# cambrian-mllm/cambrian

Measured on NVIDIA H100. Metric: train_samples_per_sec, higher is better.
Workload: dtype bf16

## Files before the change

cambrian_b200/autograd.py:

```python
from __future__ import annotations

import torch

from . import ops


def _ranged(tag):
    def deco(fn):
        def wrapped(*a, **k):
            with ops.nvtx(tag):
                return fn(*a, **k)
        wrapped.__name__ = fn.__name__
        wrapped.__doc__ = fn.__doc__
        return wrapped
    return deco


def _notify(param):
    n = getattr(param, "_cb_notify", None)
    if n is not None:
        n()


def _await(*params):
# ... 372 lines not shown
        ops.gemm(b, weight[:, D:], out=t32, accumulate=True)
        y = ops.f32_to_bf16(t32, torch.empty(t32.shape, dtype=torch.bfloat16, device=a.device))
        ctx.save_for_backward(a, b, weight)
        ctx.param = weight
        return y

    @staticmethod
    def backward(ctx, dy):
        a, b, weight = ctx.saved_tensors
        D = a.shape[1]
        dy = dy.contiguous()
        da = ops.gemm(dy, weight[:, :D], b_mn=True) if ctx.needs_input_grad[0] else None
        db = ops.gemm(dy, weight[:, D:], b_mn=True) if ctx.needs_input_grad[1] else None
        dw = None
        w_param = ctx.param
        if ctx.needs_input_grad[2] and not _frozen(w_param):
            if getattr(w_param, "main_grad", None) is not None:
                wgrad(w_param, dy, a, out_view=_slice_a(D), notify=False)
                wgrad(w_param, dy, b, out_view=_slice_b(D))
            else:
                dw = torch.cat([ops.gemm(dy, a, a_mn=True, b_mn=True), ops.gemm(dy, b, a_mn=True, b_mn=True)], 1)
        return da, db, dw


class LinearResidualFn(torch.autograd.Function):

    @staticmethod
    def forward(ctx, x, weight, residual):
        _await(weight)
        ctx.save_for_backward(x, weight)
        ctx.param = weight
        return ops.gemm(x, weight, residual=residual.contiguous())

    @staticmethod
    def backward(ctx, dy):
        x, weight = ctx.saved_tensors
        dy = dy.contiguous()
        dx = ops.gemm(dy, weight, b_mn=True) if ctx.needs_input_grad[0] else None
        dw = wgrad(ctx.param, dy, x) if ctx.needs_input_grad[1] else None
        return dx, dw, (dy if ctx.needs_input_grad[2] else None)


class NarrowLinearFn(torch.autograd.Function):

    PAD = 8

    @staticmethod
    def forward(ctx, x, weight):
        _await(weight)
        T, K = weight.shape
        if T > NarrowLinearFn.PAD:
            raise ValueError(f"NarrowLinearFn: {T} output rows > {NarrowLinearFn.PAD}")
        wpad = torch.zeros((NarrowLinearFn.PAD, K), dtype=weight.dtype, device=weight.device)
        wpad[:T].copy_(weight)
        ctx.save_for_backward(x, wpad)
        ctx.param, ctx.T = weight, T
        return ops.gemm(x, wpad)

    @staticmethod
    def backward(ctx, dy):
        x, wpad = ctx.saved_tensors
        dy = dy.contiguous()
        dx = ops.gemm(dy, wpad, b_mn=True) if ctx.needs_input_grad[0] else None
        dw = None
        if ctx.needs_input_grad[1] and not _frozen(ctx.param):
            dw = vgrad(ctx.param, ops.gemm(dy, x, a_mn=True, b_mn=True)[:ctx.T].contiguous())
        return dx, dw


class TowerCombineFn(torch.autograd.Function):

    @staticmethod
    def forward(ctx, logits, q_in, *aggs):
        aggs = [a.contiguous() for a in aggs]
        logits = logits.contiguous()
        ctx.save_for_backward(logits, *aggs)
        return ops.tower_combine_fwd(logits, aggs, q_in.contiguous())

    @staticmethod
    def backward(ctx, dout):
        logits, *aggs = ctx.saved_tensors
        dout = dout.contiguous()
        daggs, dlogits = ops.tower_combine_bwd(logits, aggs, dout)
        return (dlogits if ctx.needs_input_grad[0] else None, dout, *daggs)


class CrossAttnTowerFn(torch.autograd.Function):

    NAMES = ("q_ln_w", "q_ln_b", "q_w", "k_ln_w", "k_ln_b", "k_w", "v_ln_w", "v_ln_b", "v_w", "o_w", "pos")

    @staticmethod
    def forward(ctx, meta, q_in, feat, *tensors):
        _await(*meta["params"])
        P = dict(zip(CrossAttnTowerFn.NAMES, tensors))
        r = meta["r"]
        N = q_in.shape[0]
        nat = meta["natural"]
        windowed = nat is None
        B, q_side = (N, 1) if windowed else nat
        side = 0 if windowed else r * q_side
        masks = None if meta["mask"] is None else [meta["mask"]]
        f2 = feat.reshape(-1, feat.shape[-1])
        qn, mq, rq = ops.layernorm_fwd(q_in, P["q_ln_w"], P["q_ln_b"], 1e-5, save_stats=True)
        Q = ops.gemm(qn, P["q_w"])
        kin, mean, rstd = ops.layernorm_fwd(f2, P["k_ln_w"], P["k_ln_b"], 1e-5, pos=P["pos"], side=side, r=r, save_stats=True)
        vin = ops.layernorm_fwd(f2, P["v_ln_w"], P["v_ln_b"], 1e-5, pos=P["pos"], side=side, r=r)
        K = ops.gemm(kin, P["k_w"])
        V = ops.gemm(vin, P["v_w"])
        A, lse = ops.sva_window_attn_fwd(Q, [K], [V], masks, [r], B, q_side, need_lse=True, windowed=windowed)
        out = ops.gemm(A, P["o_w"])
        ctx.meta = meta
        ctx.dims = (N, B, q_side, windowed, side, feat.shape)
        ctx.save_for_backward(q_in, f2, qn, mq, rq, Q, kin, vin, mean, rstd, K, V, A, lse, *tensors)
        return out

    @staticmethod
    def backward(ctx, dout):
        meta = ctx.meta
        r = meta["r"]
        N, B, q_side, windowed, side, fshape = ctx.dims
        sv = ctx.saved_tensors
        q_in, f2, qn, mq, rq, Q, kin, vin, mean, rstd, K, V, A, lse = sv[:14]
        P = dict(zip(CrossAttnTowerFn.NAMES, sv[14:]))
        prm = dict(zip(CrossAttnTowerFn.NAMES, meta["params"]))
        masks = None if meta["mask"] is None else [meta["mask"]]
        g = {}
        dout = dout.contiguous()
        dA = ops.gemm(dout, P["o_w"], b_mn=True)
        g["o_w"] = wgrad(prm["o_w"], dout, A)
        dQ, (dK,), (dV,) = ops.sva_window_attn_bwd(Q, A, dA, lse, [K], [V], masks, [r], B, q_side, windowed=windowed)
        dqn = ops.gemm(dQ, P["q_w"], b_mn=True)
        g["q_w"] = wgrad(prm["q_w"], dQ, qn)
        dq_in, dgq, dbq = ops.layernorm_bwd(dqn, q_in, P["q_ln_w"], mq, rq)
        g["q_ln_w"], g["q_ln_b"] = vgrad(prm["q_ln_w"], dgq), vgrad(prm["q_ln_b"], dbq)
        dkin = ops.gemm(dK, P["k_w"], b_mn=True)
        g["k_w"] = wgrad(prm["k_w"], dK, kin)
        dvin = ops.gemm(dV, P["v_w"], b_mn=True)
        g["v_w"] = wgrad(prm["v_w"], dV, vin)
        dxk, dgk, dbk = ops.layernorm_bwd(dkin, f2, P["k_ln_w"], mean, rstd, pos=P["pos"], side=side, r=r)
        dxv, dgv, dbv = ops.layernorm_bwd(dvin, f2, P["v_ln_w"], mean, rstd, pos=P["pos"], side=side, r=r, dres=dxk)
        g["k_ln_w"], g["k_ln_b"] = vgrad(prm["k_ln_w"], dgk), vgrad(prm["k_ln_b"], dbk)
        g["v_ln_w"], g["v_ln_b"] = vgrad(prm["v_ln_w"], dgv), vgrad(prm["v_ln_b"], dbv)
        dp = ops.pos_grad(dxv, dxv.shape[0] // (r * r), r, r) if windowed else ops.pos_grad(dxv, B, r * q_side, r)
        g["pos"] = vgrad(prm["pos"], dp)
        return (None, dq_in, dxv.view(fshape), *[g[n] for n in CrossAttnTowerFn.NAMES])


class DecoderLayerFn(torch.autograd.Function):
    _nvtx = "DecoderLayer"

    """x [B,S,H] -> x'.  Parameters: input_ln, qkv_w (fused [ (nh+2nkv)*hd, H ]), o_w, post_ln, gu_w (fused [2I, H]), down_w.

    meta = dict(nh, nkv, hd, eps, hf_cast, cos, sin, pos (int64 [B*S]), kmask (bool [B,S] or None), params (6 Parameters),
                recompute (bool: keep only x and redo the forward in backward — per-layer activation checkpointing))
    """

    @staticmethod
    def _forward(meta, x, ln1, qkv_w, o_w, ln2, gu_w, down_w, keep, need_out=True):
        B, S, H = x.shape
        nh, nkv, hd = meta["nh"], meta["nkv"], meta["hd"]
        rows = B * S
        x2 = x.reshape(rows, H)
        h, rstd1 = ops.rmsnorm_fwd(x2, ln1, meta["eps"], meta["hf_cast"], save_stats=True)
        qkv = ops.gemm(h, qkv_w)
        ops.rope_(qkv, meta["pos"], meta["cos"], meta["sin"], nh + nkv, hd)
        q = qkv[:, : nh * hd].view(B, S, nh, hd)
        k = qkv[:, nh * hd:(nh + nkv) * hd].view(B, S, nkv, hd)
        v = qkv[:, (nh + nkv) * hd:].view(B, S, nkv, hd)
        attn, lse = ops.attn_fwd(q, k, v, causal=True, kmask=meta["kmask"], need_lse=True)
        attn2 = attn.view(rows, nh * hd)
        x1 = ops.gemm(attn2, o_w, residual=x2)
        h2, rstd2 = ops.rmsnorm_fwd(x1, ln2, meta["eps"], meta["hf_cast"], save_stats=True)
        gu, act = ops.mlp_gate_up(h2, gu_w)
        saved = (rstd1, qkv, attn, lse, x1, rstd2, gu, act) if keep else None
        if not need_out:
            return None, saved
        out = ops.gemm(act, down_w, residual=x1)
        return out.view(B, S, H), saved

    @staticmethod
    @_ranged("decoder_layer.fwd")
    def forward(ctx, meta, x, ln1, q_w, k_w, v_w, o_w, ln2, gate_w, up_w, down_w):
        keep = not meta["recompute"]
        _await(*meta["params"])
        qkv_w, gu_w = meta["qkv_w"], meta["gu_w"]
        out, saved = DecoderLayerFn._forward(meta, x, ln1, qkv_w, o_w, ln2, gu_w, down_w, keep)
        ctx.meta = meta
        if keep:
            ctx.save_for_backward(x, ln1, qkv_w, o_w, ln2, gu_w, down_w, *saved)
        else:
            ctx.save_for_backward(x, ln1, qkv_w, o_w, ln2, gu_w, down_w)
        return out

    @staticmethod
    @_ranged("decoder_layer.bwd")
    def backward(ctx, dout):
        meta = ctx.meta
        sv = ctx.saved_tensors
        x, ln1, qkv_w, o_w, ln2, gu_w, down_w = sv[:7]
        if meta["recompute"]:
            _, saved = DecoderLayerFn._forward(meta, x, ln1, qkv_w, o_w, ln2, gu_w, down_w, True, need_out=False)
        else:
            saved = sv[7:]
        rstd1, qkv, attn, lse, x1, rstd2, gu, act = saved
        p_ln1, p_qkv, p_o, p_ln2, p_gu, p_down = meta["params"]
        B, S, H = x.shape
        nh, nkv, hd = meta["nh"], meta["nkv"], meta["hd"]
        rows = B * S
        I = gu_w.shape[0] // 2
        x2 = x.reshape(rows, H)
        dx2 = dout.reshape(rows, H).contiguous()
        h2 = ops.rmsnorm_fwd(x1, ln2, meta["eps"], meta["hf_cast"])
        dact = ops.gemm(dx2, down_w, b_mn=True)
        g_down = wgrad(p_down, dx2, act)
        del act
        dgu = torch.empty_like(gu)
        ops.swiglu_bwd(dact, gu[:, :I], gu[:, I:], dgu[:, :I], dgu[:, I:])
        del dact
        dh2 = ops.gemm(dgu, gu_w, b_mn=True)
        g_gu = wgrad(p_gu, dgu, h2)
        del dgu, h2
        dx1, dg2 = ops.rmsnorm_bwd(dh2, x1, ln2, rstd2, dres=dx2)
        g_ln2 = vgrad(p_ln2, dg2)
        attn2 = attn.view(rows, nh * hd)
        dattn = ops.gemm(dx1, o_w, b_mn=True)
        g_o = wgrad(p_o, dx1, attn2)
        dqkv = torch.empty_like(qkv)
        q = qkv[:, : nh * hd].view(B, S, nh, hd)
        k = qkv[:, nh * hd:(nh + nkv) * hd].view(B, S, nkv, hd)
        v = qkv[:, (nh + nkv) * hd:].view(B, S, nkv, hd)
        ops.attn_bwd(q, k, v, attn, dattn.view(B, S, nh, hd), lse, causal=True, kmask=meta["kmask"],
                     dq=dqkv[:, : nh * hd].view(B, S, nh, hd), dk=dqkv[:, nh * hd:(nh + nkv) * hd].view(B, S, nkv, hd),
                     dv=dqkv[:, (nh + nkv) * hd:].view(B, S, nkv, hd))
        ops.rope_(dqkv, meta["pos"], meta["cos"], meta["sin"], nh + nkv, hd, inverse=True)
        h = ops.rmsnorm_fwd(x2, ln1, meta["eps"], meta["hf_cast"])
        dh = ops.gemm(dqkv, qkv_w, b_mn=True)
        g_qkv = wgrad(p_qkv, dqkv, h)
        del dqkv, h
        dx, dg1 = ops.rmsnorm_bwd(dh, x2, ln1, rstd1, dres=dx1)
        g_ln1 = vgrad(p_ln1, dg1)
        gq = gk = gv = gg = gup = None
        if g_qkv is not None:
            gq, gk, gv = g_qkv[: nh * hd], g_qkv[nh * hd:(nh + nkv) * hd], g_qkv[(nh + nkv) * hd:]
        if g_gu is not None:
            gg, gup = g_gu[:I], g_gu[I:]
        return None, dx.view(B, S, H), g_ln1, gq, gk, gv, g_o, g_ln2, gg, gup, g_down


class EmbedSpliceFn(torch.autograd.Function):

    @staticmethod
    def forward(ctx, meta, embed_w, img, newline):
        ids, img_start, q_side = meta["ids"], meta["img_start"], meta["q_side"]
        _await(*meta["params"])
        ctx.meta = meta
        ctx.has_img = img is not None
        ctx.vshape = embed_w.shape
        return ops.embed_splice(ids, img_start, embed_w, img, newline, q_side)

    @staticmethod
    def backward(ctx, dout):
        meta = ctx.meta
        p_embed, p_newline = meta["params"]
        dout = dout.contiguous()
        d_embed_ret = None
        tgt = None
        if ctx.needs_input_grad[1]:
            mg = getattr(p_embed, "main_grad", None)
            if mg is not None:
                fresh = getattr(p_embed, "_cb_fresh", None)
                if fresh is not None and "all" not in fresh:
                    mg.zero_()
                    fresh.add("all")
                tgt = mg
            else:
                tgt = torch.zeros(ctx.vshape, dtype=torch.bfloat16, device=dout.device)
                d_embed_ret = tgt
        d_img, d_nl_rows = ops.embed_splice_bwd(dout, meta["ids"], meta["img_start"], None, meta["q_side"], ctx.has_img)
        if tgt is not None:
            ops.embed_grad_sorted(dout, meta["ids"], meta["img_start"] if ctx.has_img else None, tgt, meta["q_side"])
        if tgt is not None and d_embed_ret is None:
            _notify(p_embed)
        d_nl = None
        if ctx.has_img and ctx.needs_input_grad[3]:
            d_nl = vgrad(p_newline, ops.group_colsum(d_nl_rows, 1).view(-1))
        return None, d_embed_ret, d_img, d_nl


class LMHeadLossFn(torch.autograd.Function):
    _nvtx = "LMHeadLoss"

    """cambrian_llama.py:402-422: lm_head -> logits.float() -> shift -> CrossEntropyLoss(mean over non-ignored), computed
    in row chunks so the [B*S, V] logits are never resident at once; the backward GEMMs run inside the forward (the
    per-chunk (softmax - onehot) overwrites the chunk's logits), so the only saved tensor is dhidden."""

    @staticmethod
    @_ranged("lm_head_loss.fwd")
    def forward(ctx, meta, hidden, weight):
        labels = meta["shift_labels"]
        rows, H = hidden.reshape(-1, hidden.shape[-1]).shape
        h2 = hidden.reshape(rows, H)
        V = weight.shape[0]
        dev = hidden.device
        chunk = meta.get("chunk", 4096)
        n_valid = meta["n_valid"]
        inv_dev = meta.get("inv_count_dev")
        train = meta["train"]
        p_w = meta["params"][0]
        _await(p_w)
        need_dw = train and not _frozen(p_w)
        ranges = meta.get("label_ranges")
        dh_full = None
        if ranges is not None:
            ranges = [(int(a), int(b)) for a, b in ranges if b > a]
            n_rows = sum(b - a for a, b in ranges)
            hc = torch.empty((max(n_rows, 1), H), dtype=h2.dtype, device=dev)
            lc = torch.full((max(n_rows, 1),), -100, dtype=labels.dtype, device=dev)
            o = 0
            for a, b in ranges:
                hc[o:o + b - a].copy_(h2[a:b])
                lc[o:o + b - a].copy_(labels[a:b])
                o += b - a
            if train:
                dh_full = torch.zeros_like(h2)
            h2, labels, rows = hc, lc, max(n_rows, 1)
        loss_rows = torch.empty(rows, dtype=torch.float32, device=dev)
        acc = torch.zeros(2, dtype=torch.float32, device=dev)
        dh = torch.empty_like(h2) if train else None
        gscale = float(meta.get("loss_scale", 1.0)) / (max(n_valid, 1) if n_valid is not None else 1)
        logits = torch.empty((min(chunk, rows), V), dtype=torch.bfloat16, device=dev)
        dw_local = None
        if need_dw and getattr(p_w, "main_grad", None) is None:
            dw_local = torch.empty_like(weight)
        for r0 in range(0, rows, chunk):
            r1 = min(rows, r0 + chunk)
            lg = logits[: r1 - r0]
            ops.gemm(h2[r0:r1], weight, out=lg)
            ops.cross_entropy(lg, labels[r0:r1], loss_rows[r0:r1], acc, gscale, train,
                              scale_dev=inv_dev if n_valid is None else None)
            if train:
                ops.gemm(lg, weight, b_mn=True, out=dh[r0:r1])
                if not need_dw:
                    pass
                elif dw_local is None:
                    wgrad(p_w, lg, h2[r0:r1], notify=False)
                else:
                    ops.gemm(lg, h2[r0:r1], a_mn=True, b_mn=True, out=dw_local, accumulate=r0 > 0)
        if need_dw and dw_local is None:
            _notify(p_w)
        if dh_full is not None:
            o = 0
            for a, b in ranges:
                dh_full[a:b].copy_(dh[o:o + b - a])
                o += b - a
            dh = dh_full
        ctx.train = train
        ctx.hshape = hidden.shape
# ... 69 lines not shown
```

cambrian_b200/csrc/attention.cu:

```cuda
#include "common.cuh"
#include <cudaTypedefs.h>
#include <type_traits>

namespace cb {

int make_tmap_bf16_4d(CUtensorMap* out, const void* base, uint64_t d0, uint64_t d1, uint64_t d2, uint64_t d3,
                      uint64_t s1, uint64_t s2, uint64_t s3, uint32_t box_rows);

constexpr float LOG2E = 1.4426950408889634f;

struct AttnParams {
  bf16* o;
  long long o_bs, o_ss;
  float* lse;
  const uint8_t* kmask;
  int B, nh, nkv, Sq, Skv, hd, causal;
  float scale_log2;
};

template <int N>
__device__ __forceinline__ bool keys_all_valid(const uint8_t* km, int k0) {
  constexpr int PER = N / 32;
  static_assert(PER == 2 || PER == 4, "64- or 128-key tiles");
  const uint8_t* kp = km + k0 + PER * (threadIdx.x & 31);
  uint32_t w = 0;
  if (!(reinterpret_cast<uintptr_t>(kp) & (PER - 1))) {
    w = PER == 4 ? *reinterpret_cast<const uint32_t*>(kp) : *reinterpret_cast<const uint16_t*>(kp);
  } else {
#pragma unroll
    for (int i = 0; i < PER; ++i) w |= (uint32_t)kp[i] << (8 * i);
  }
  bool ok = true;
#pragma unroll
  for (int i = 0; i < PER; ++i) ok = ok && ((w >> (8 * i)) & 0xffu);
  return __all_sync(0xffffffffu, ok);
}

struct TileIdx {
  int t, h, b;
};
__device__ __forceinline__ TileIdx tile_index(int heads, int B) {
  const int hb = heads * B;
  const int rem = (int)blockIdx.x % hb;
  return {(int)blockIdx.x / hb, rem % heads, rem / heads};
}

template <int HDP>
struct FwdCfg {
  static constexpr int ATOMS = (HDP + 63) / 64;
  static constexpr int TILE = ATOMS * 16384;
  static constexpr int STAGES = 3;
  static constexpr int SMEM = TILE * (1 + 2 * STAGES) + 1024 + 256;
};

template <int HDP>
__global__ void __launch_bounds__(288, 1)
attn_fwd_kernel(const __grid_constant__ CUtensorMap tmQ, const __grid_constant__ CUtensorMap tmK,
                const __grid_constant__ CUtensorMap tmV, AttnParams p) {
  using Cfg = FwdCfg<HDP>;
  constexpr int STAGES = Cfg::STAGES;
  extern __shared__ uint8_t smem_raw[];
  const uint32_t base = (smem_u32(smem_raw) + 1023u) & ~1023u;
  const uint32_t sQ = base;
  const uint32_t sK = sQ + Cfg::TILE;
  const uint32_t sV = sK + STAGES * Cfg::TILE;
  const uint32_t bars = sV + STAGES * Cfg::TILE;
  const uint32_t q_full = bars;
  auto k_full = [&](int s) { return bars + 8u * (1 + s); };
  auto v_full = [&](int s) { return bars + 8u * (1 + STAGES + s); };
  auto kv_empty = [&](int s) { return bars + 8u * (1 + 2 * STAGES + s); };

  const int warp = threadIdx.x >> 5, lane = threadIdx.x & 31;
  const int q_tiles = (p.Sq + 127) / 128;
  const TileIdx ti = tile_index(p.nh, p.B);
  const int qt = q_tiles - 1 - ti.t;
  const int h = ti.h, b = ti.b;
  const int hk = h / (p.nh / p.nkv);
  const int q0 = qt * 128;
  const int kv_tiles_all = (p.Skv + 127) / 128;
  const int coff = p.Skv - p.Sq;
  int n_tiles = kv_tiles_all;
  if (p.causal) {
    const int last_key = q0 + 127 + coff;
    n_tiles = min(kv_tiles_all, last_key / 128 + 1);
    if (n_tiles < 1) n_tiles = 1;
  }

  if (warp == 8 && lane == 0) {
    tma_prefetch_desc(&tmQ);
    tma_prefetch_desc(&tmK);
    tma_prefetch_desc(&tmV);
    mbar_init(q_full, 1);
    for (int s = 0; s < STAGES; ++s) {
      mbar_init(k_full(s), 1);
      mbar_init(v_full(s), 1);
      mbar_init(kv_empty(s), 2);
    }
    mbar_fence_init();
  }
  __syncthreads();

  if (warp == 8) {
    if (lane == 0) {
      mbar_arrive_expect_tx(q_full, Cfg::TILE);
#pragma unroll
      for (int a = 0; a < Cfg::ATOMS; ++a) tma_load_4d(sQ + a * 16384, &tmQ, q_full, a * 64, h, q0, b);
      int st = 0;
      uint32_t ph = 0;
      for (int j = 0; j < n_tiles; ++j) {
        mbar_wait(kv_empty(st), ph ^ 1u);
        mbar_arrive_expect_tx(k_full(st), Cfg::TILE);
#pragma unroll
        for (int a = 0; a < Cfg::ATOMS; ++a)
          tma_load_4d(sK + st * Cfg::TILE + a * 16384, &tmK, k_full(st), a * 64, hk, j * 128, b);
        mbar_arrive_expect_tx(v_full(st), Cfg::TILE);
#pragma unroll
        for (int a = 0; a < Cfg::ATOMS; ++a)
          tma_load_4d(sV + st * Cfg::TILE + a * 16384, &tmV, v_full(st), a * 64, hk, j * 128, b);
        if (++st == STAGES) { st = 0; ph ^= 1u; }
      }
    }
    return;
  }

  const int wg = warp >> 2;
  const bool wg_leader = (threadIdx.x & 127) == 0;
  const int rloc = wg * 64 + (warp & 3) * 16 + (lane >> 2);
  const int cq = 2 * (lane & 3);
  const uint8_t* km = p.kmask ? p.kmask + (size_t)b * p.Skv : nullptr;
  float o[HDP / 2];
#pragma unroll
  for (int i = 0; i < HDP / 2; ++i) o[i] = 0.f;
  float m_run[2] = {-INFINITY, -INFINITY}, l_run[2] = {0.f, 0.f};
  mbar_wait(q_full, 0);
  int st = 0;
  uint32_t ph = 0;
  for (int j = 0; j < n_tiles; ++j) {
    const int k0 = j * 128;
    float s[64];
    mbar_wait(k_full(st), ph);
    const uint32_t kb = sK + st * Cfg::TILE;
    wgmma_fence();
#pragma unroll
    for (int kk = 0; kk < HDP / 16; ++kk) {
      const uint32_t off = (kk >> 2) * 16384 + (kk & 3) * 32;
      WgmmaSS<128, 0, 0>::mma(s, make_smem_desc_sw128(sQ + wg * 8192 + off, 0, 1024),
                              make_smem_desc_sw128(kb + off, 0, 1024), kk ? 1u : 0u);
    }
    wgmma_commit();
    bool full_tile = k0 + 128 <= p.Skv && (!p.causal || k0 + 127 <= q0 + wg * 64 + coff);
    if (full_tile && km) full_tile = keys_all_valid<128>(km, k0);
    wgmma_wait<0>();
    reg_fence(s);
    float mx[2] = {-INFINITY, -INFINITY};
#pragma unroll
    for (int jj = 0; jj < 16; ++jj) {
#pragma unroll
      for (int e = 0; e < 4; ++e) {
        float v = s[4 * jj + e] * p.scale_log2;
        if (!full_tile) {
          const int key = k0 + 8 * jj + cq + (e & 1);
          const int qi = q0 + rloc + 8 * (e >> 1);
          const bool ok = key < p.Skv && (!p.causal || key <= qi + coff) && (!km || km[key]);
          v = ok ? v : -INFINITY;
        }
        s[4 * jj + e] = v;
        mx[e >> 1] = fmaxf(mx[e >> 1], v);
      }
    }
    float corr[2], mref[2];
#pragma unroll
    for (int r = 0; r < 2; ++r) {
      mx[r] = fmaxf(mx[r], __shfl_xor_sync(0xffffffffu, mx[r], 1));
      mx[r] = fmaxf(mx[r], __shfl_xor_sync(0xffffffffu, mx[r], 2));
      const float m_new = fmaxf(m_run[r], mx[r]);
      mref[r] = m_new == -INFINITY ? 0.f : m_new;
      corr[r] = fast_exp2(m_run[r] - mref[r]);
      m_run[r] = m_new;
      l_run[r] *= corr[r];
    }
#pragma unroll
    for (int jj = 0; jj < HDP / 8; ++jj) {
#pragma unroll
      for (int e = 0; e < 4; ++e) o[4 * jj + e] *= corr[e >> 1];
    }
    uint32_t pa[8][4];
#pragma unroll
    for (int jj = 0; jj < 16; ++jj) {
      float pv[4];
#pragma unroll
      for (int e = 0; e < 4; ++e) {
        pv[e] = fast_exp2(s[4 * jj + e] - mref[e >> 1]);
        l_run[e >> 1] += pv[e];
      }
      pa[jj >> 1][(jj & 1) * 2 + 0] = pack_bf16x2(pv[0], pv[1]);
      pa[jj >> 1][(jj & 1) * 2 + 1] = pack_bf16x2(pv[2], pv[3]);
    }
    mbar_wait(v_full(st), ph);
    const uint32_t vb = sV + st * Cfg::TILE;
    reg_fence(o);
    wgmma_fence();
#pragma unroll
    for (int kk = 0; kk < 8; ++kk)
      WgmmaRS<HDP, 1>::mma(o, pa[kk], make_smem_desc_sw128(vb + kk * 2048, 16384, 1024), 1u);
    wgmma_commit();
    wgmma_wait<0>();
    reg_fence(o);
    if (wg_leader) mbar_arrive(kv_empty(st));
    if (++st == STAGES) { st = 0; ph ^= 1u; }
  }
#pragma unroll
  for (int r = 0; r < 2; ++r) {
    float l = l_run[r];
    l += __shfl_xor_sync(0xffffffffu, l, 1);
    l += __shfl_xor_sync(0xffffffffu, l, 2);
    const int qi = q0 + rloc + 8 * r;
    if (qi >= p.Sq) continue;
    const float inv = l > 0.f ? 1.f / l : 0.f;
    bf16* op = p.o + (long long)b * p.o_bs + (long long)qi * p.o_ss + (long long)h * p.hd;
#pragma unroll
    for (int jj = 0; jj < HDP / 8; ++jj) {
      const int d = 8 * jj + cq;
      if (d < p.hd)
        *reinterpret_cast<__nv_bfloat162*>(op + d) = __floats2bfloat162_rn(o[4 * jj + 2 * r] * inv, o[4 * jj + 2 * r + 1] * inv);
    }
    if (p.lse && (lane & 3) == 0)
      p.lse[((long long)b * p.nh + h) * p.Sq + qi] = l > 0.f ? m_run[r] + log2f(l) : INFINITY;
  }
}

__global__ void attn_delta_kernel(const bf16* __restrict__ o, const bf16* __restrict__ d_o, float* __restrict__ delta,
                                  int B, int S, int nh, int hd, long long o_bs, long long o_ss, long long do_bs,
                                  long long do_ss) {
  const int lph = hd >> 3;
  const int hpw = 32 / lph;
  const long long w = (blockIdx.x * (long long)blockDim.x + threadIdx.x) >> 5;
  const int lane = threadIdx.x & 31;
  const long long total = (long long)B * S * nh;
  const long long idx = w * hpw + lane / lph;
  const int sub = lane % lph;
  float acc = 0.f;
  if (idx < total) {
    const int h = (int)(idx % nh);
    const long long t = idx / nh;
    const int s = (int)(t % S);
    const int b = (int)(t / S);
    const bf16* op = o + b * o_bs + s * o_ss + (long long)h * hd + sub * 8;
    const bf16* gp = d_o + b * do_bs + s * do_ss + (long long)h * hd + sub * 8;
    float a[8], g[8];
    unpack8(ldg_nc(op), a);
    unpack8(ldg_nc(gp), g);
#pragma unroll
    for (int e = 0; e < 8; ++e) acc += a[e] * g[e];
  }
  for (int off = lph >> 1; off > 0; off >>= 1) acc += __shfl_xor_sync(0xffffffffu, acc, off);
  if (idx < total && sub == 0) {
    const int h = (int)(idx % nh);
    const long long t = idx / nh;
    delta[((long long)(t / S) * nh + h) * S + (t % S)] = acc;
  }
}

struct AttnBwdParams {
  bf16* dq;
  bf16* dk;
  bf16* dv;
  long long dq_bs, dq_ss, dk_bs, dk_ss, dv_bs, dv_ss;
  const float* lse;
  const float* delta;
  const uint8_t* kmask;
  int B, nh, nkv, Sq, Skv, hd, causal;
  float scale_log2, scale;
};

template <int HDP>
struct BwdCfg {
  static constexpr int ATOMS = HDP / 64;
  static constexpr int KTILE = ATOMS * 16384;
  static constexpr int QTILE = ATOMS * 8192;
  static constexpr int STAGES = 4;
  static constexpr int SMEM = 2 * KTILE + 2 * STAGES * QTILE + STAGES * 512 + 1024 + 256;
};

template <int HDP>
__global__ void __launch_bounds__(384, 1)
attn_bwd_kernel(const __grid_constant__ CUtensorMap tmQ, const __grid_constant__ CUtensorMap tmK,
                const __grid_constant__ CUtensorMap tmV, const __grid_constant__ CUtensorMap tmdO, AttnBwdParams p) {
  using Cfg = BwdCfg<HDP>;
  constexpr int STAGES = Cfg::STAGES;
  extern __shared__ uint8_t smem_raw[];
  const uint32_t base = (smem_u32(smem_raw) + 1023u) & ~1023u;
  const uint32_t sK = base;
  const uint32_t sV = sK + Cfg::KTILE;
  const uint32_t sQ = sV + Cfg::KTILE;
  const uint32_t sdO = sQ + STAGES * Cfg::QTILE;
  const uint32_t sLD = sdO + STAGES * Cfg::QTILE;
  const uint32_t bars = sLD + STAGES * 512;
  const uint32_t kv_full = bars;
  auto qd_full = [&](int s) { return bars + 8u * (1 + s); };
  auto qd_empty = [&](int s) { return bars + 8u * (1 + STAGES + s); };
  float* ld_stage = reinterpret_cast<float*>(smem_raw + (sLD - smem_u32(smem_raw)));

  const int warp = threadIdx.x >> 5, lane = threadIdx.x & 31;
  const TileIdx ti = tile_index(p.nkv, p.B);
// ... 112 lines not shown
      for (int jj = 0; jj < 8; ++jj) {
        float pv[4], dsv[4];
#pragma unroll
        for (int c = 0; c < 2; ++c) {
          const int qc = 8 * jj + cq + c;
          const float L = ld[qc], D = ld[64 + qc];
#pragma unroll
          for (int r = 0; r < 2; ++r) {
            const int e = 2 * r + c;
            bool vis = true;
            if (!decltype(full_tile)::value)
              vis = qi0 + qc < p.Sq && key_ok[r] && (!p.causal || k0 + kr + 8 * r <= qi0 + qc + coff);
            const float pe = vis ? fast_exp2(fmaf(sT[4 * jj + e], p.scale_log2, -L)) : 0.f;
            pv[e] = pe;
            dsv[e] = pe * (dpT[4 * jj + e] - D);
          }
        }
        pa[jj >> 1][(jj & 1) * 2 + 0] = pack_bf16x2(pv[0], pv[1]);
        pa[jj >> 1][(jj & 1) * 2 + 1] = pack_bf16x2(pv[2], pv[3]);
        da[jj >> 1][(jj & 1) * 2 + 0] = pack_bf16x2(dsv[0], dsv[1]);
        da[jj >> 1][(jj & 1) * 2 + 1] = pack_bf16x2(dsv[2], dsv[3]);
      }
    };
    if (full)
      grads(std::true_type());
    else
      grads(std::false_type());
    reg_fence(dv);
    reg_fence(dk);
    wgmma_fence();
#pragma unroll
    for (int kk = 0; kk < 4; ++kk) {
      WgmmaRS<HDP, 1>::mma(dv, pa[kk], make_smem_desc_sw128(dob + kk * 2048, 8192, 1024), 1u);
      WgmmaRS<HDP, 1>::mma(dk, da[kk], make_smem_desc_sw128(qb + kk * 2048, 8192, 1024), 1u);
    }
    wgmma_commit();
    wgmma_wait<0>();
    reg_fence(dv);
    reg_fence(dk);
    if (lane == 0) mbar_arrive(qd_empty(st));
    if (++st == STAGES) { st = 0; ph ^= 1u; }
  }
#pragma unroll
  for (int r = 0; r < 2; ++r) {
    const int kidx = k0 + kr + 8 * r;
    if (kidx >= p.Skv) continue;
    bf16* dkp = p.dk + (long long)b * p.dk_bs + (long long)kidx * p.dk_ss + (long long)g * p.hd;
    bf16* dvp = p.dv + (long long)b * p.dv_bs + (long long)kidx * p.dv_ss + (long long)g * p.hd;
#pragma unroll
    for (int jj = 0; jj < HDP / 8; ++jj) {
      const int d = 8 * jj + cq;
      *reinterpret_cast<__nv_bfloat162*>(dkp + d) =
          __floats2bfloat162_rn(dk[4 * jj + 2 * r] * p.scale, dk[4 * jj + 2 * r + 1] * p.scale);
      *reinterpret_cast<__nv_bfloat162*>(dvp + d) = __floats2bfloat162_rn(dv[4 * jj + 2 * r], dv[4 * jj + 2 * r + 1]);
    }
  }
}

template <int HDP>
struct DqCfg {
  static constexpr int ATOMS = HDP / 64;
  static constexpr int QTILE = ATOMS * 16384;
  static constexpr int KTILE = ATOMS * 8192;
  static constexpr int STAGES = 4;
  static constexpr int SMEM = 2 * QTILE + 2 * STAGES * KTILE + 1024 + 256;
};

template <int HDP>
__global__ void __launch_bounds__(288, 1)
attn_bwd_dq_kernel(const __grid_constant__ CUtensorMap tmQ, const __grid_constant__ CUtensorMap tmK,
                   const __grid_constant__ CUtensorMap tmV, const __grid_constant__ CUtensorMap tmdO, AttnBwdParams p) {
  using Cfg = DqCfg<HDP>;
  constexpr int STAGES = Cfg::STAGES;
  extern __shared__ uint8_t smem_raw[];
  const uint32_t base = (smem_u32(smem_raw) + 1023u) & ~1023u;
  const uint32_t sQ = base;
  const uint32_t sdO = sQ + Cfg::QTILE;
  const uint32_t sK = sdO + Cfg::QTILE;
  const uint32_t sV = sK + STAGES * Cfg::KTILE;
  const uint32_t bars = sV + STAGES * Cfg::KTILE;
  const uint32_t q_full = bars;
  auto kv_full = [&](int s) { return bars + 8u * (1 + s); };
  auto kv_empty = [&](int s) { return bars + 8u * (1 + STAGES + s); };

  const int warp = threadIdx.x >> 5, lane = threadIdx.x & 31;
  const int q_tiles = (p.Sq + 127) / 128;
  const TileIdx ti = tile_index(p.nh, p.B);
  const int qt = q_tiles - 1 - ti.t;
  const int h = ti.h, b = ti.b;
  const int hk = h / (p.nh / p.nkv);
  const int q0 = qt * 128;
  const int coff = p.Skv - p.Sq;
  const int kv_tiles_all = (p.Skv + 63) / 64;
  int n_tiles = kv_tiles_all;
  if (p.causal) n_tiles = max(1, min(kv_tiles_all, (q0 + 127 + coff) / 64 + 1));

  if (warp == 8 && lane == 0) {
    tma_prefetch_desc(&tmQ);
    tma_prefetch_desc(&tmK);
    tma_prefetch_desc(&tmV);
    tma_prefetch_desc(&tmdO);
    mbar_init(q_full, 1);
    for (int s = 0; s < STAGES; ++s) {
      mbar_init(kv_full(s), 1);
      mbar_init(kv_empty(s), 2);
    }
    mbar_fence_init();
  }
  __syncthreads();

  if (warp == 8) {
    if (lane == 0) {
      mbar_arrive_expect_tx(q_full, 2 * Cfg::QTILE);
#pragma unroll
      for (int a = 0; a < Cfg::ATOMS; ++a) {
        tma_load_4d(sQ + a * 16384, &tmQ, q_full, a * 64, h, q0, b);
        tma_load_4d(sdO + a * 16384, &tmdO, q_full, a * 64, h, q0, b);
      }
      int st = 0;
      uint32_t ph = 0;
      for (int j = 0; j < n_tiles; ++j) {
        mbar_wait(kv_empty(st), ph ^ 1u);
        mbar_arrive_expect_tx(kv_full(st), 2 * Cfg::KTILE);
#pragma unroll
        for (int a = 0; a < Cfg::ATOMS; ++a) {
          tma_load_4d(sK + st * Cfg::KTILE + a * 8192, &tmK, kv_full(st), a * 64, hk, j * 64, b);
          tma_load_4d(sV + st * Cfg::KTILE + a * 8192, &tmV, kv_full(st), a * 64, hk, j * 64, b);
        }
        if (++st == STAGES) { st = 0; ph ^= 1u; }
      }
    }
    return;
  }

  const int wg = warp >> 2;
  const bool wg_leader = (threadIdx.x & 127) == 0;
  const int rloc = wg * 64 + (warp & 3) * 16 + (lane >> 2);
  const int cq = 2 * (lane & 3);
  const int wq0 = q0 + wg * 64 + (warp & 3) * 16;
  const uint8_t* km = p.kmask ? p.kmask + (size_t)b * p.Skv : nullptr;
  const float* lse = p.lse + ((long long)b * p.nh + h) * p.Sq;
  const float* dlt = p.delta + ((long long)b * p.nh + h) * p.Sq;
  int qi[2];
  float L[2], D[2];
#pragma unroll
  for (int r = 0; r < 2; ++r) {
    qi[r] = q0 + rloc + 8 * r;
    L[r] = qi[r] < p.Sq ? __ldg(lse + qi[r]) : 0.f;
    D[r] = qi[r] < p.Sq ? __ldg(dlt + qi[r]) : 0.f;
  }
  float dq[HDP / 2];
#pragma unroll
  for (int i = 0; i < HDP / 2; ++i) dq[i] = 0.f;
  mbar_wait(q_full, 0);
  int st = 0;
  uint32_t ph = 0;
  for (int j = 0; j < n_tiles; ++j) {
    const int k0 = j * 64;
    mbar_wait(kv_full(st), ph);
    const uint32_t kb = sK + st * Cfg::KTILE, vb = sV + st * Cfg::KTILE;
    float s[32], dp[32];
    wgmma_fence();
#pragma unroll
    for (int kk = 0; kk < HDP / 16; ++kk) {
      const uint32_t qoff = wg * 8192 + (kk >> 2) * 16384 + (kk & 3) * 32, koff = (kk >> 2) * 8192 + (kk & 3) * 32;
      WgmmaSS<64, 0, 0>::mma(s, make_smem_desc_sw128(sQ + qoff, 0, 1024), make_smem_desc_sw128(kb + koff, 0, 1024),
                             kk ? 1u : 0u);
    }
#pragma unroll
    for (int kk = 0; kk < HDP / 16; ++kk) {
      const uint32_t qoff = wg * 8192 + (kk >> 2) * 16384 + (kk & 3) * 32, koff = (kk >> 2) * 8192 + (kk & 3) * 32;
      WgmmaSS<64, 0, 0>::mma(dp, make_smem_desc_sw128(sdO + qoff, 0, 1024), make_smem_desc_sw128(vb + koff, 0, 1024),
                             kk ? 1u : 0u);
    }
    wgmma_commit();
    bool full = k0 + 64 <= p.Skv && wq0 + 16 <= p.Sq && (!p.causal || k0 + 63 <= wq0 + coff);
    if (full && km) full = keys_all_valid<64>(km, k0);
    wgmma_wait<0>();
    reg_fence(s);
    reg_fence(dp);
    uint32_t da[4][4];
    auto grads = [&](auto full_tile) {
#pragma unroll
      for (int jj = 0; jj < 8; ++jj) {
        float dsv[4];
#pragma unroll
        for (int e = 0; e < 4; ++e) {
          const int r = e >> 1, key = k0 + 8 * jj + cq + (e & 1);
          bool vis = true;
          if (!decltype(full_tile)::value)
            vis = qi[r] < p.Sq && key < p.Skv && (!p.causal || key <= qi[r] + coff) && (!km || km[key]);
          const float pe = vis ? fast_exp2(fmaf(s[4 * jj + e], p.scale_log2, -L[r])) : 0.f;
          dsv[e] = pe * (dp[4 * jj + e] - D[r]);
        }
        da[jj >> 1][(jj & 1) * 2 + 0] = pack_bf16x2(dsv[0], dsv[1]);
        da[jj >> 1][(jj & 1) * 2 + 1] = pack_bf16x2(dsv[2], dsv[3]);
      }
    };
    if (full)
      grads(std::true_type());
    else
      grads(std::false_type());
    reg_fence(dq);
    wgmma_fence();
#pragma unroll
    for (int kk = 0; kk < 4; ++kk)
      WgmmaRS<HDP, 1>::mma(dq, da[kk], make_smem_desc_sw128(kb + kk * 2048, 8192, 1024), 1u);
    wgmma_commit();
    wgmma_wait<0>();
    reg_fence(dq);
    if (wg_leader) mbar_arrive(kv_empty(st));
    if (++st == STAGES) { st = 0; ph ^= 1u; }
  }
#pragma unroll
  for (int r = 0; r < 2; ++r) {
    if (qi[r] >= p.Sq) continue;
    bf16* dqp = p.dq + (long long)b * p.dq_bs + (long long)qi[r] * p.dq_ss + (long long)h * p.hd;
#pragma unroll
    for (int jj = 0; jj < HDP / 8; ++jj)
      *reinterpret_cast<__nv_bfloat162*>(dqp + 8 * jj + cq) =
          __floats2bfloat162_rn(dq[4 * jj + 2 * r] * p.scale, dq[4 * jj + 2 * r + 1] * p.scale);
  }
}

static PFN_cuTensorMapEncodeTiled_v12000 encode_fn() {
  static PFN_cuTensorMapEncodeTiled_v12000 fn = nullptr;
  if (!fn) {
    void* ptr = nullptr;
    cudaDriverEntryPointQueryResult q;
    if (cudaGetDriverEntryPoint("cuTensorMapEncodeTiled", &ptr, cudaEnableDefault, &q) == cudaSuccess &&
        q == cudaDriverEntryPointSuccess)
      fn = reinterpret_cast<PFN_cuTensorMapEncodeTiled_v12000>(ptr);
  }
  return fn;
}

int make_tmap_bf16_4d(CUtensorMap* out, const void* base, uint64_t d0, uint64_t d1, uint64_t d2, uint64_t d3,
                      uint64_t s1, uint64_t s2, uint64_t s3, uint32_t box_rows) {
  auto fn = encode_fn();
  if (!fn) return set_error(CB_ERR_CUDA, "cuTensorMapEncodeTiled entry point not available");
  if ((reinterpret_cast<uintptr_t>(base) & 15u) || (s1 % 8) || (s2 % 8) || (d3 > 1 && (s3 % 8)))
    return set_error(CB_ERR_INVALID, "attention: operands must be 16-byte aligned with strides %% 8 == 0");
  cuuint64_t dims[4] = {d0, d1, d2, d3};
  cuuint64_t strides[3] = {s1 * 2, s2 * 2, (d3 > 1 ? s3 : s2 * d2) * 2};
  cuuint32_t box[4] = {64, 1, box_rows, 1};
  cuuint32_t estr[4] = {1, 1, 1, 1};
  CUresult r = fn(out, CU_TENSOR_MAP_DATA_TYPE_BFLOAT16, 4, const_cast<void*>(base), dims, strides, box, estr,
                  CU_TENSOR_MAP_INTERLEAVE_NONE, CU_TENSOR_MAP_SWIZZLE_128B, CU_TENSOR_MAP_L2_PROMOTION_L2_256B,
                  CU_TENSOR_MAP_FLOAT_OOB_FILL_NONE);
  if (r == CUDA_ERROR_INVALID_CONTEXT) {
    cudaFree(0);
    r = fn(out, CU_TENSOR_MAP_DATA_TYPE_BFLOAT16, 4, const_cast<void*>(base), dims, strides, box, estr,
           CU_TENSOR_MAP_INTERLEAVE_NONE, CU_TENSOR_MAP_SWIZZLE_128B, CU_TENSOR_MAP_L2_PROMOTION_L2_256B,
           CU_TENSOR_MAP_FLOAT_OOB_FILL_NONE);
  }
  if (r != CUDA_SUCCESS) return set_error(CB_ERR_CUDA, "cuTensorMapEncodeTiled(4d) failed (%d)", (int)r);
  return CB_OK;
}

static int hd_padded(int hd) { return (hd + 15) / 16 * 16; }

template <int HDP>
static int launch_fwd(const CUtensorMap& tq, const CUtensorMap& tk, const CUtensorMap& tv, const AttnParams& p,
                      cudaStream_t st) {
  using Cfg = FwdCfg<HDP>;
  auto kern = attn_fwd_kernel<HDP>;
  static bool attr = false;
  if (!attr) {
    cudaError_t e = cudaFuncSetAttribute(kern, cudaFuncAttributeMaxDynamicSharedMemorySize, Cfg::SMEM);
    if (e != cudaSuccess) return set_error(CB_ERR_CUDA, "attn fwd smem attr: %s", cudaGetErrorString(e));
    attr = true;
  }
  kern<<<(p.Sq + 127) / 128 * p.nh * p.B, 288, Cfg::SMEM, st>>>(tq, tk, tv, p);
  CB_CUDA_LAUNCH_CHECK("attn_fwd");
  return CB_OK;
}

int attn_fwd_launch(const void* q, const void* k, const void* v, void* o, float* lse, const void* kmask, int B,
                    int nh, int nkv, int Sq, int Skv, int hd, long long q_bs, long long q_ss, long long k_bs,
                    long long k_ss, long long v_bs, long long v_ss, long long o_bs, long long o_ss, float scale,
                    int causal, cudaStream_t st) {
  CB_CHECK_ARG(B > 0 && nh > 0 && nkv > 0 && Sq > 0 && Skv > 0, "attention: empty problem");
  CB_CHECK_ARG(nh % nkv == 0, "attention: nh=%d not a multiple of nkv=%d", nh, nkv);
  CB_CHECK_ARG(hd % 8 == 0 && hd <= 128, "attention: head_dim=%d must be a multiple of 8 and <= 128", hd);
  CB_CHECK_ARG(o_ss % 8 == 0 && o_bs % 8 == 0 && !(reinterpret_cast<uintptr_t>(o) & 15u),
               "attention: output must be 16-byte aligned with strides %% 8 == 0");
  CUtensorMap tq, tk, tv;
  int rc;
  if ((rc = make_tmap_bf16_4d(&tq, q, hd, nh, Sq, B, hd, q_ss, q_bs, 128))) return rc;
  if ((rc = make_tmap_bf16_4d(&tk, k, hd, nkv, Skv, B, hd, k_ss, k_bs, 128))) return rc;
  if ((rc = make_tmap_bf16_4d(&tv, v, hd, nkv, Skv, B, hd, v_ss, v_bs, 128))) return rc;
  AttnParams p;
  p.o = (bf16*)o; p.o_bs = o_bs; p.o_ss = o_ss; p.lse = lse; p.kmask = (const uint8_t*)kmask;
  p.B = B; p.nh = nh; p.nkv = nkv; p.Sq = Sq; p.Skv = Skv; p.hd = hd; p.causal = causal;
  p.scale_log2 = scale * LOG2E;
  const int hdp = hd_padded(hd);
  if (hdp <= 64) return launch_fwd<64>(tq, tk, tv, p, st);
  if (hdp <= 80) return launch_fwd<80>(tq, tk, tv, p, st);
  if (hdp <= 96) return launch_fwd<96>(tq, tk, tv, p, st);
  return launch_fwd<128>(tq, tk, tv, p, st);
}

template <int HDP>
static int launch_bwd(const CUtensorMap& tq, const CUtensorMap& tk, const CUtensorMap& tv, const CUtensorMap& tdo,
                      const AttnBwdParams& p, cudaStream_t st) {
  using Cfg = BwdCfg<HDP>;
  auto kern = attn_bwd_kernel<HDP>;
  static bool attr = false;
  if (!attr) {
    cudaError_t e = cudaFuncSetAttribute(kern, cudaFuncAttributeMaxDynamicSharedMemorySize, Cfg::SMEM);
    if (e != cudaSuccess) return set_error(CB_ERR_CUDA, "attn bwd smem attr: %s", cudaGetErrorString(e));
    attr = true;
  }
  kern<<<(p.Skv + 127) / 128 * p.nkv * p.B, 384, Cfg::SMEM, st>>>(tq, tk, tv, tdo, p);
  CB_CUDA_LAUNCH_CHECK("attn_bwd");
  return CB_OK;
}

template <int HDP>
static int launch_bwd_dq(const CUtensorMap& tq, const CUtensorMap& tk, const CUtensorMap& tv, const CUtensorMap& tdo,
                         const AttnBwdParams& p, cudaStream_t st) {
  using Cfg = DqCfg<HDP>;
  auto kern = attn_bwd_dq_kernel<HDP>;
  static bool attr = false;
  if (!attr) {
    cudaError_t e = cudaFuncSetAttribute(kern, cudaFuncAttributeMaxDynamicSharedMemorySize, Cfg::SMEM);
    if (e != cudaSuccess) return set_error(CB_ERR_CUDA, "attn bwd dq smem attr: %s", cudaGetErrorString(e));
    attr = true;
  }
  kern<<<(p.Sq + 127) / 128 * p.nh * p.B, 288, Cfg::SMEM, st>>>(tq, tk, tv, tdo, p);
// ... 49 lines not shown
```

Measured before the change: 7.897.

## Save attention output in checkpointing and prefetch key-mask words a tile ahead

Under per-layer recompute, the decoder layer now keeps the attention output, lse and x1 and re-runs only the RMSNorm→QKV→RoPE and RMSNorm→gate/up parts in backward. This skips recomputing the flash attention forward and the o-projection, at the cost of more activation memory. Separately, the attention forward and backward kernels load the key-mask word for the next tile one iteration early, so the global load overlaps with the MMA rather than sitting on the critical path.

```diff
diff --git a/cambrian_b200/autograd.py b/cambrian_b200/autograd.py
--- a/cambrian_b200/autograd.py
+++ b/cambrian_b200/autograd.py
@@ -548,29 +548,38 @@
     """x [B,S,H] -> x'.  Parameters: input_ln, qkv_w (fused [ (nh+2nkv)*hd, H ]), o_w, post_ln, gu_w (fused [2I, H]), down_w.
 
     meta = dict(nh, nkv, hd, eps, hf_cast, cos, sin, pos (int64 [B*S]), kmask (bool [B,S] or None), params (6 Parameters),
-                recompute (bool: keep only x and redo the forward in backward — per-layer activation checkpointing))
+                recompute (bool: keep x, the attention output, lse and x1, and redo the RMSNorm -> QKV -> RoPE and
+                RMSNorm -> gate/up ends of the layer in backward — per-layer activation checkpointing))
     """
 
     @staticmethod
-    def _forward(meta, x, ln1, qkv_w, o_w, ln2, gu_w, down_w, keep, need_out=True):
+    def _qkv(meta, x2, ln1, qkv_w):
+        h, rstd1 = ops.rmsnorm_fwd(x2, ln1, meta["eps"], meta["hf_cast"], save_stats=True)
+        qkv = ops.gemm(h, qkv_w)
+        ops.rope_(qkv, meta["pos"], meta["cos"], meta["sin"], meta["nh"] + meta["nkv"], meta["hd"])
+        return rstd1, qkv
+
+    @staticmethod
+    def _gate_up(meta, x1, ln2, gu_w):
+        h2, rstd2 = ops.rmsnorm_fwd(x1, ln2, meta["eps"], meta["hf_cast"], save_stats=True)
+        gu, act = ops.mlp_gate_up(h2, gu_w)
+        return rstd2, gu, act
+
+    @staticmethod
+    def _forward(meta, x, ln1, qkv_w, o_w, ln2, gu_w, down_w, keep):
         B, S, H = x.shape
         nh, nkv, hd = meta["nh"], meta["nkv"], meta["hd"]
         rows = B * S
         x2 = x.reshape(rows, H)
-        h, rstd1 = ops.rmsnorm_fwd(x2, ln1, meta["eps"], meta["hf_cast"], save_stats=True)
-        qkv = ops.gemm(h, qkv_w)
-        ops.rope_(qkv, meta["pos"], meta["cos"], meta["sin"], nh + nkv, hd)
+        rstd1, qkv = DecoderLayerFn._qkv(meta, x2, ln1, qkv_w)
         q = qkv[:, : nh * hd].view(B, S, nh, hd)
         k = qkv[:, nh * hd:(nh + nkv) * hd].view(B, S, nkv, hd)
         v = qkv[:, (nh + nkv) * hd:].view(B, S, nkv, hd)
         attn, lse = ops.attn_fwd(q, k, v, causal=True, kmask=meta["kmask"], need_lse=True)
         attn2 = attn.view(rows, nh * hd)
         x1 = ops.gemm(attn2, o_w, residual=x2)
-        h2, rstd2 = ops.rmsnorm_fwd(x1, ln2, meta["eps"], meta["hf_cast"], save_stats=True)
-        gu, act = ops.mlp_gate_up(h2, gu_w)
-        saved = (rstd1, qkv, attn, lse, x1, rstd2, gu, act) if keep else None
-        if not need_out:
-            return None, saved
+        rstd2, gu, act = DecoderLayerFn._gate_up(meta, x1, ln2, gu_w)
+        saved = (rstd1, qkv, attn, lse, x1, rstd2, gu, act) if keep else (attn, lse, x1)
         out = ops.gemm(act, down_w, residual=x1)
         return out.view(B, S, H), saved
 
@@ -582,10 +591,7 @@
         qkv_w, gu_w = meta["qkv_w"], meta["gu_w"]
         out, saved = DecoderLayerFn._forward(meta, x, ln1, qkv_w, o_w, ln2, gu_w, down_w, keep)
         ctx.meta = meta
-        if keep:
-            ctx.save_for_backward(x, ln1, qkv_w, o_w, ln2, gu_w, down_w, *saved)
-        else:
-            ctx.save_for_backward(x, ln1, qkv_w, o_w, ln2, gu_w, down_w)
+        ctx.save_for_backward(x, ln1, qkv_w, o_w, ln2, gu_w, down_w, *saved)
         return out
 
     @staticmethod
@@ -595,10 +601,11 @@
         sv = ctx.saved_tensors
         x, ln1, qkv_w, o_w, ln2, gu_w, down_w = sv[:7]
         if meta["recompute"]:
-            _, saved = DecoderLayerFn._forward(meta, x, ln1, qkv_w, o_w, ln2, gu_w, down_w, True, need_out=False)
+            attn, lse, x1 = sv[7:]
+            rstd1, qkv = DecoderLayerFn._qkv(meta, x.reshape(-1, x.shape[-1]), ln1, qkv_w)
+            rstd2, gu, act = DecoderLayerFn._gate_up(meta, x1, ln2, gu_w)
         else:
-            saved = sv[7:]
-        rstd1, qkv, attn, lse, x1, rstd2, gu, act = saved
+            rstd1, qkv, attn, lse, x1, rstd2, gu, act = sv[7:]
         p_ln1, p_qkv, p_o, p_ln2, p_gu, p_down = meta["params"]
         B, S, H = x.shape
         nh, nkv, hd = meta["nh"], meta["nkv"], meta["hd"]
diff --git a/cambrian_b200/csrc/attention.cu b/cambrian_b200/csrc/attention.cu
--- a/cambrian_b200/csrc/attention.cu
+++ b/cambrian_b200/csrc/attention.cu
@@ -19,7 +19,7 @@
 };
 
 template <int N>
-__device__ __forceinline__ bool keys_all_valid(const uint8_t* km, int k0) {
+__device__ __forceinline__ uint32_t keys_word(const uint8_t* km, int k0) {
   constexpr int PER = N / 32;
   static_assert(PER == 2 || PER == 4, "64- or 128-key tiles");
   const uint8_t* kp = km + k0 + PER * (threadIdx.x & 31);
@@ -30,6 +30,12 @@
 #pragma unroll
     for (int i = 0; i < PER; ++i) w |= (uint32_t)kp[i] << (8 * i);
   }
+  return w;
+}
+
+template <int N>
+__device__ __forceinline__ bool keys_all_set(uint32_t w) {
+  constexpr int PER = N / 32;
   bool ok = true;
 #pragma unroll
   for (int i = 0; i < PER; ++i) ok = ok && ((w >> (8 * i)) & 0xffu);
@@ -132,11 +138,14 @@
 #pragma unroll
   for (int i = 0; i < HDP / 2; ++i) o[i] = 0.f;
   float m_run[2] = {-INFINITY, -INFINITY}, l_run[2] = {0.f, 0.f};
+  uint32_t kw_next = km && 128 <= p.Skv ? keys_word<128>(km, 0) : 0u;
   mbar_wait(q_full, 0);
   int st = 0;
   uint32_t ph = 0;
   for (int j = 0; j < n_tiles; ++j) {
     const int k0 = j * 128;
+    const uint32_t kw = kw_next;
+    if (km && j + 1 < n_tiles && k0 + 256 <= p.Skv) kw_next = keys_word<128>(km, k0 + 128);
     float s[64];
     mbar_wait(k_full(st), ph);
     const uint32_t kb = sK + st * Cfg::TILE;
@@ -149,7 +158,7 @@
     }
     wgmma_commit();
     bool full_tile = k0 + 128 <= p.Skv && (!p.causal || k0 + 127 <= q0 + wg * 64 + coff);
-    if (full_tile && km) full_tile = keys_all_valid<128>(km, k0);
+    if (full_tile && km) full_tile = keys_all_set<128>(kw);
     wgmma_wait<0>();
     reg_fence(s);
     float mx[2] = {-INFINITY, -INFINITY};
@@ -568,11 +577,14 @@
   float dq[HDP / 2];
 #pragma unroll
   for (int i = 0; i < HDP / 2; ++i) dq[i] = 0.f;
+  uint32_t kw_next = km && 64 <= p.Skv ? keys_word<64>(km, 0) : 0u;
   mbar_wait(q_full, 0);
   int st = 0;
   uint32_t ph = 0;
   for (int j = 0; j < n_tiles; ++j) {
     const int k0 = j * 64;
+    const uint32_t kw = kw_next;
+    if (km && j + 1 < n_tiles && k0 + 128 <= p.Skv) kw_next = keys_word<64>(km, k0 + 64);
     mbar_wait(kv_full(st), ph);
     const uint32_t kb = sK + st * Cfg::KTILE, vb = sV + st * Cfg::KTILE;
     float s[32], dp[32];
@@ -591,7 +603,7 @@
     }
     wgmma_commit();
     bool full = k0 + 64 <= p.Skv && wq0 + 16 <= p.Sq && (!p.causal || k0 + 63 <= wq0 + coff);
-    if (full && km) full = keys_all_valid<64>(km, k0);
+    if (full && km) full = keys_all_set<64>(kw);
     wgmma_wait<0>();
     reg_fence(s);
     reg_fence(dp);
```

Measured after the change: 8.216 (median of 6 runs). 4.0% higher.
